# mcdermatt/ICET

Hardware: NVIDIA B200
Metric: registrations/s (64-ch, 75x24 vox, 7 it) (higher is better)
Workload: dtype f32

## Files before the change

### icet_b200/csrc/chunk.cuh

```cuda
#pragma once

thread_local std::string g_err;
int fail(int code, const std::string& msg) {
  g_err = msg;
  return code;
}
#define CK(call)                                                                              \
  do {                                                                                        \
    cudaError_t e_ = (call);                                                                  \
    if (e_ != cudaSuccess)                                                                    \
      return fail(ICET_B200_E_CUDA, std::string(#call) + ": " + cudaGetErrorString(e_));      \
  } while (0)

constexpr int FPB = 21;
constexpr int FP_LIM = (1 << FPB);
constexpr unsigned FULL = 0xffffffffu;
constexpr uint32_t F_STAT1 = 1u;
constexpr uint32_t F_ACTIVE2 = 2u;
constexpr int SORT_SMEM = 4096;
constexpr int NQ = 12;
constexpr int CLUSTER_WARPS = 4;
constexpr int WSORT_MAX = 1024;
constexpr int HUGE_MIN = 32768;
constexpr int HUGE_SLOTS = 64;
constexpr int HUGE_NB = 32768;
constexpr int HUGE_SPLIT = 128;
constexpr uint32_t CLS_CELL = 0x003fffffu;
constexpr uint32_t CLS_IN = 0x00400000u;
constexpr uint32_t CLS_ACTIVE = 0x00800000u;
constexpr uint32_t CLS_NONE = 0x003fffffu;

struct PairDesc {
  const float* s1;
  const float* s2;
  int n1, ld1, n2, ld2;
};

__host__ __device__ __forceinline__ int fp_bits(int n) {
  const unsigned m = (unsigned)(n > 2 ? n : 2) - 1u;
#ifdef __CUDA_ARCH__
  const int lg = 32 - __clz(m);
#else
  const int lg = 32 - __builtin_clz(m);
#endif
  const int b = (62 - lg) / 2;
  return b < 12 ? 12 : (b > 23 ? 23 : b);
}
struct FixPt {
  float fs;
  int fl;
};
// ... 152 lines not shown
  return ok != 0;
}
__device__ __forceinline__ void mbar_wait(unsigned long long* bar, unsigned parity) {
  if (mbar_try_wait(bar, parity)) return;
  unsigned long long t0 = 0;
  for (unsigned spin = 1; !mbar_try_wait(bar, parity); spin++) {
    if ((spin & 1023u) == 0u) {
      unsigned long long t;
      asm volatile("mov.u64 %0, %%globaltimer;" : "=l"(t));
      if (t0 == 0) t0 = t;
      else if (t - t0 > 20000000000ull) __trap();
    }
  }
}

__device__ __forceinline__ uint32_t opaque_u32(uint32_t v) {
  uint32_t r;
  asm volatile("mov.u32 %0, %1;" : "=r"(r) : "r"(v));
  return r;
}
__device__ __forceinline__ float lds_f32(uint32_t a) {
  float v;
  asm volatile("ld.shared.f32 %0, [%1];" : "=f"(v) : "r"(a) : "memory");
  return v;
}
__device__ __forceinline__ uint32_t lds_u32(uint32_t a) {
  uint32_t v;
  asm volatile("ld.shared.u32 %0, [%1];" : "=r"(v) : "r"(a) : "memory");
  return v;
}
__device__ __forceinline__ void sts_u32(uint32_t a, uint32_t v) {
  asm volatile("st.shared.u32 [%0], %1;" ::"r"(a), "r"(v) : "memory");
}
```

### icet_b200/csrc/kernels_pass2.cuh

```cuda
#pragma once

constexpr float INC_MAX_SA = 1.0e-3f;
constexpr float INC_MAX_SB = 0.05f;

struct Pass2Mode {
  bool rebuild;
  int set;
  float fs2;
  int fl2;
  float SA, SB, C;
  const float* trbp;
  unsigned long long* accp;
};

__device__ __forceinline__ float rec2_round_re(float r) {
  return __uint_as_float((__float_as_uint(r * 1.000001f) + 0xffffu) & 0xffff0000u);
}
__device__ __forceinline__ uint2 rec2_pack(float u, float re , uint32_t cls) {
  return make_uint2((__float_as_uint(fmaxf(u, 0.f)) & 0xffffff00u) | (cls & 0xffu), __float_as_uint(re) | (cls >> 8));
}
__device__ __forceinline__ float rec2_u(uint2 v) { return __uint_as_float(v.x & 0xffffff00u); }
__device__ __forceinline__ float rec2_re(uint2 v) { return __uint_as_float(v.y & 0xffff0000u); }
__device__ __forceinline__ uint32_t rec2_cls(uint2 v) { return (v.x & 0xffu) | ((v.y & 0xffffu) << 8); }

// ... 198 lines not shown
  class_move(md.accp, recs, md, old, cls, 0.f, 0.f, 0.f, nz);
  ck.pm[pair].zcls = (int)cls;
}

__device__ __forceinline__ void flush_run2(unsigned long long* accp, int cell, int nb, int nin, int sx, int sy, int sz,
                                           long long pxx, long long pxy, long long pxz, long long pyy, long long pyz,
                                           long long pzz) {
  if (cell < 0) return;
  unsigned long long* q = accp + (size_t)cell * NQ;
  red_add(q, (unsigned long long)nb);
  if (nin == 0) return;
  red_add(q + 1, (unsigned long long)nin);
  red_add(q + 2, (unsigned long long)(long long)sx);
  red_add(q + 3, (unsigned long long)(long long)sy);
  red_add(q + 4, (unsigned long long)(long long)sz);
  red_add(q + 5, (unsigned long long)pxx);
  red_add(q + 6, (unsigned long long)pxy);
  red_add(q + 7, (unsigned long long)pxz);
  red_add(q + 8, (unsigned long long)pyy);
  red_add(q + 9, (unsigned long long)pyz);
  red_add(q + 10, (unsigned long long)pzz);
}

template <int K>
__device__ __forceinline__ void pass2_request_tile(int4* went, const float* src, size_t ld, int cnt, unsigned long long* mbar) {
  float* tx = reinterpret_cast<float*>(went);
  const unsigned bytes = (unsigned)((cnt + 3) & ~3) * 4u;
  mbar_expect_tx(mbar, 3u * bytes);
  bulk_g2s(tx, src, bytes, mbar);
  bulk_g2s(tx + 32 * K, src + ld, bytes, mbar);
  bulk_g2s(tx + 64 * K, src + 2 * ld, bytes, mbar);
}

template <int K, int RD = K, bool ANCH = false>
__device__ __forceinline__ void pass2_warp_tile(const Chunk& ck, int4* went, unsigned long long* mbar, unsigned& mphase,
                                                bool requested, const float* tab, const CellRec* recs, const float* tr,
                                                const Pass2Mode& md, const float* pog, size_t ld, int n, int w0, uint2* mrec,
                                                int* violations, const float4* anch = nullptr) {
  static_assert(K <= 16, "list entries keep the point's index within the tile in 9 bits");
  const int lane = threadIdx.x & 31;
  if (w0 >= n) return;
  const int cnt = min(n - w0, 32 * K);
  const float4* tth = reinterpret_cast<const float4*>(tab);
  const float4* tph = tth + ck.nT + 2;
  const unsigned lt = (1u << lane) - 1u;
  unsigned long long* accp = md.accp;
  const uint32_t sb = opaque_u32(smem_u32(went));
  const uint32_t sbl = sb + 4u * lane;
  constexpr uint32_t PL = 128u * K;
  constexpr uint32_t LO = 3u * PL;
  uint2* rp = mrec + w0;
  if (md.rebuild) {
    if (!requested) {
      __syncwarp();
      if (lane == 0) pass2_request_tile<K>(went, pog + w0, ld, cnt, mbar);
    }
    mbar_wait(mbar, mphase);
    mphase ^= 1u;
    int nact = 0;
#pragma unroll(K % 4 == 0 ? 4 : 2)
    for (int j = 0; j < K; j++) {
      const int li = j * 32 + lane;
      uint32_t cls = 0u;
      if (li < cnt) {
        const float x = lds_f32(sbl + 128u * j), y = lds_f32(sbl + 128u * j + PL), z = lds_f32(sbl + 128u * j + 2u * PL);
        float2 mg;
        point_eval2_fast(ck, tth, tph, recs, tr, 0.f, 0.f, x, y, z, cls, mg);
        if (violations) {
          uint32_t cx;
          float2 mx;
          point_eval2(ck, tth, tph, recs, tr, 0.f, 0.f, x, y, z, cx, mx);
          if (cx != cls) atomicAdd(violations + 1, 1);
        }
        rp[li] = rec2_pack(mg.x, mg.y, cls);
      }
      const bool act = (cls & CLS_ACTIVE) != 0;
      const unsigned am = __ballot_sync(FULL, act);
      if (act) sts_u32(sb + LO + 4u * (nact + __popc(am & lt)), ((uint32_t)li << 23) | (cls & (CLS_CELL | CLS_IN)));
      nact += __popc(am);
    }
    __syncwarp();
    const int q = ((nact + 31) >> 5) | 1;
    const int e0 = lane * q, e1 = min(nact, e0 + q);
    int cur = -1, nb = 0, nin = 0, sx = 0, sy = 0, sz = 0;
    long long pxx = 0, pxy = 0, pxz = 0, pyy = 0, pyz = 0, pzz = 0;
    float ax = 0.f, ay = 0.f, az = 0.f, sc = 0.f;
#pragma unroll 2
    for (int e = e0; e < e1; e++) {
      const unsigned v = lds_u32(sb + LO + 4u * e);
      const int c = (int)(v & CLS_CELL);
      if (c != cur) {
        flush_run2(accp, cur, nb, nin, sx, sy, sz, pxx, pxy, pxz, pyy, pyz, pzz);
        cur = c;
        nb = nin = sx = sy = sz = 0;
        pxx = pxy = pxz = pyy = pyz = pzz = 0;
        if (ANCH) {
          const float4 an = __ldg(anch + cur);
          ax = an.x; ay = an.y; az = an.z; sc = an.w;
        } else {
          vox_anchor2(recs, cur, tr, md.fs2, ax, ay, az, sc);
        }
      }
      nb++;
      if (v & CLS_IN) {
        const uint32_t pa = sb + 4u * (v >> 23);
        int fx, fy, fz;
        fix2(lds_f32(pa), lds_f32(pa + PL), lds_f32(pa + 2u * PL), ax, ay, az, sc, md.fl2, fx, fy, fz);
        nin++;
        sx += fx; sy += fy; sz += fz;
        pxx += (long long)fx * fx; pxy += (long long)fx * fy; pxz += (long long)fx * fz;
        pyy += (long long)fy * fy; pyz += (long long)fy * fz; pzz += (long long)fz * fz;
      }
    }
    flush_run2(accp, cur, nb, nin, sx, sy, sz, pxx, pxy, pxz, pyy, pyz, pzz);
    __syncwarp();
    return;
  }
  int nre = 0;
  constexpr int R = RD;
  static_assert(K % RD == 0, "rows per load group must divide the tile");
#pragma unroll 1
  for (int j0 = 0; j0 < K; j0 += R) {
    uint2 rv[R];
#pragma unroll
    for (int g = 0; g < R; g++) {
      const int li = (j0 + g) * 32 + lane;
      rv[g] = make_uint2(0x7f000000u, 0u);
      if (li < cnt) rv[g] = __ldcg(rp + li);
    }
#pragma unroll
    for (int g = 0; g < R; g++) {
      const int li = (j0 + g) * 32 + lane;
      const bool stable = fmaf(rec2_re(rv[g]), md.SA, md.C) < rec2_u(rv[g]);
      const bool redo = li < cnt && (!stable || violations != nullptr);
      const unsigned rm = __ballot_sync(FULL, redo);
      if (redo) sts_u32(sb + LO + 4u * (nre + __popc(rm & lt)), stable ? ((uint32_t)li | 0x80000000u) : (uint32_t)li);
      nre += __popc(rm);
    }
  }
  if (nre == 0) return;
  const bool staged = nre * 8 > cnt;
  __syncwarp();
  if (staged) {
    if (lane == 0) pass2_request_tile<K>(went, pog + w0, ld, cnt, mbar);
    mbar_wait(mbar, mphase);
    mphase ^= 1u;
  }
  for (int e0 = 0; e0 < nre; e0 += 32) {
    const int e = e0 + lane;
    if (e < nre) {
      const uint32_t le = lds_u32(sb + LO + 4u * e);
      const bool was_stable = (le & 0x80000000u) != 0;
      const int li = (int)(le & 0x7fffffffu);
      float x, y, z;
      if (staged) {
        x = lds_f32(sb + 4u * li); y = lds_f32(sb + 4u * li + PL); z = lds_f32(sb + 4u * li + 2u * PL);
      } else {
        const float* pp = pog + w0 + li;
        x = __ldg(pp); y = __ldg(pp + ld); z = __ldg(pp + 2 * ld);
      }
      const uint32_t old = rec2_cls(__ldcg(rp + li));
      uint32_t cls;
      float2 mg;
      point_eval2_fast(ck, tth, tph, recs, tr, md.SA, md.SB, x, y, z, cls, mg);
      if (violations) {
        uint32_t cx;
        float2 mx;
        point_eval2(ck, tth, tph, recs, tr, md.SA, md.SB, x, y, z, cx, mx);
        if (cx != cls) atomicAdd(violations + 1, 1);
      }
      rp[li] = rec2_pack(mg.x, mg.y, cls);
      if (cls != old) {
        if (was_stable) atomicAdd(violations, 1);
        class_move(accp, recs, md, old, cls, x, y, z, 1);
      }
    }
  }
  __syncwarp();
}

__device__ __forceinline__ void load_pass2_mode(const Chunk& ck, int pair, Pass2Mode& md) {
  const PairMode* pm = ck.pm + pair;
  const int4 h = __ldcg(reinterpret_cast<const int4*>(pm));
  md.rebuild = h.y != 0;
  md.set = h.x;
  const FixPt fp = fix_point(__ldg(&ck.desc[pair].n2));
  md.fs2 = fp.fs;
  md.fl2 = fp.fl;
  md.SA = __int_as_float(h.z);
  md.C = __int_as_float(h.w);
  md.SB = __ldcg(&pm->SB);
  md.trbp = pm->TRb;
  md.accp = ck.acc + ((size_t)h.x * ck.npairs + pair) * ck.ncell * NQ;
}

template <int K = PASS_K, int MINB = PASS_MINB>
__global__ void __launch_bounds__(PASS_THREADS, MINB) k_pass2(const Chunk ck) {
  pdl_prologue();
  extern __shared__ __align__(16) unsigned char smem_raw[];
  __shared__ unsigned long long s_mbar[PASS_WARPS];
  int4* ent = reinterpret_cast<int4*>(smem_raw);
  float* tab = reinterpret_cast<float*>(smem_raw + PASS_WARPS * pass_wslots(K) * 16);
  const int pair = blockIdx.y;
  const int n = ck.n2c[pair];
  const int tile0 = blockIdx.x * pass_tile_points(K);
  if (tile0 >= n && blockIdx.x != 0) return;
  const int warp = threadIdx.x >> 5, lane = threadIdx.x & 31;
  int4* went = ent + warp * pass_wslots(K);
  const int w0 = tile0 + warp * 32 * K;
  const float* pog = ck.pog + (size_t)pair * 3 * ck.n2max;
  Pass2Mode md;
  load_pass2_mode(ck, pair, md);
  if (lane == 0) mbar_init(&s_mbar[warp], 1);
  __syncwarp();
  const bool requested = md.rebuild && w0 < n;
  if (requested && lane == 0) pass2_request_tile<K>(went, pog + w0, (size_t)ck.n2max, min(n - w0, 32 * K), &s_mbar[warp]);
  const float* tabp = ck.binrec;
  if (md.rebuild) {
    const int ntab = pass_tab_floats(ck.nT, ck.nP);
    for (int k = threadIdx.x; k < ntab; k += PASS_THREADS) tab[k] = __ldg(ck.binrec + k);
    tabp = tab;
    __syncthreads();
  }
  float tr[12];
  {
    const float4* tp = reinterpret_cast<const float4*>(ck.TR + (size_t)pair * 12);
    const float4 a = __ldcg(tp), b = __ldcg(tp + 1), c = __ldcg(tp + 2);
    tr[0] = a.x; tr[1] = a.y; tr[2] = a.z; tr[3] = a.w; tr[4] = b.x; tr[5] = b.y; tr[6] = b.z; tr[7] = b.w;
    tr[8] = c.x; tr[9] = c.y; tr[10] = c.z; tr[11] = c.w;
  }
  const CellRec* recs = ck.rec + (size_t)pair * ck.ncell;
  unsigned mphase = 0u;
  pass2_warp_tile<K, K, true>(ck, went, &s_mbar[warp], mphase, requested, tabp, recs, tr, md, pog, (size_t)ck.n2max, n, w0,
                              ck.mrec + (size_t)pair * ck.n2max,
                              (ck.flags & ICET_B200_FLAG_VERIFY_INCREMENTAL) ? &ck.res[pair].reserved[0] : nullptr,
                              ck.anch + (size_t)pair * ck.ncell);
  if (blockIdx.x == 0 && threadIdx.x == 0)
    pass2_dropped_returns(ck, reinterpret_cast<const float4*>(tabp), reinterpret_cast<const float4*>(tabp) + ck.nT + 2, recs,
                          tr, md, pair, ck.nz2[pair]);
}
```

### icet_b200/csrc/kernels_pass.cuh

```cuda
#pragma once
constexpr int PASS_THREADS = 256;
constexpr int PASS_WARPS = PASS_THREADS / 32;
constexpr int PASS_K = 12;
constexpr int PASS_MINB = 4;
constexpr int PASS_K_SMALL = 4;

__host__ __device__ constexpr int pass_wslots(int K) { return 32 * K; }
__host__ __device__ constexpr int pass_tile_points(int K) { return PASS_WARPS * 32 * K; }
__host__ __device__ inline int pass_tab_floats(int nT, int nP) { return 6 * (nT + nP + 4); }
__host__ __device__ inline int pass_smem_bytes(int nT, int nP, int K) {
  return PASS_WARPS * pass_wslots(K) * 16 + pass_tab_floats(nT, nP) * 4;
}

__device__ __forceinline__ int bin_box(float a, const float4* rec, const icet::BinTable& bt, bool& inbox) {
  int k = __float2int_rz(fminf(a, bt.acap) * bt.scale);
  float4 e = rec[k];
  if (a < e.x || a >= e.y) {
    k += (a < e.x) ? -1 : 1;
    e = rec[k];
  }
  inbox = a >= e.z && a <= e.w;
  return k < bt.nb ? k : (k == bt.nb ? 0 : bt.sbin);
}

// ... 70 lines not shown
template <bool SCAN2, int K, int PF = 2, int G = 1>
__device__ __forceinline__ void pass_warp_tile(const Chunk& ck, int4* went ,
                                               const float* tab, const CellRec* recs, const float* tr,
                                               const float* px_, size_t ld, int n, int w0, FixPt fp,
                                               unsigned long long* accp, unsigned long long* dbg_stamp = nullptr,
                                               const int32_t* s1_cell = nullptr, const float* s1_th = nullptr,
                                               const float* s1_ph = nullptr) {
  const int lane = threadIdx.x & 31;
  if (w0 >= n) return;
  const float4* tth = reinterpret_cast<const float4*>(tab);
  const float4* tph = tth + ck.nT + 2;
  const unsigned lt = (1u << lane) - 1u;
  int nin_tile = 0;
  if (!SCAN2) {
    constexpr int R = (K % 4 == 0) ? 4 : ((K % 2 == 0) ? 2 : 1);
#pragma unroll 1
    for (int j0 = 0; j0 < K; j0 += R) {
      int cid[R];
      float rr[R], tt[R], pp[R];
#pragma unroll
      for (int g = 0; g < R; g++) {
        const int i = w0 + (j0 + g) * 32 + lane;
        cid[g] = -1; rr[g] = 0.f; tt[g] = 0.f; pp[g] = 0.f;
        if (i < n) { cid[g] = __ldg(s1_cell + i); rr[g] = __ldg(px_ + i); tt[g] = __ldg(s1_th + i); pp[g] = __ldg(s1_ph + i); }
      }
      float4 ra[R];
#pragma unroll
      for (int g = 0; g < R; g++) {
        ra[g] = make_float4(0.f, 0.f, 0.f, 0.f);
        if (cid[g] >= 0) ra[g] = __ldg(reinterpret_cast<const float4*>(recs + (cid[g] & ~CELL_INBOX)));
      }
#pragma unroll
      for (int g = 0; g < R; g++) {
        const bool in = cid[g] >= 0 && (cid[g] & CELL_INBOX) && (__float_as_uint(ra[g].z) & F_STAT1) && rr[g] >= ra[g].x &&
                        rr[g] <= ra[g].y;
        const unsigned im = __ballot_sync(FULL, in);
        if (in)
          went[nin_tile + __popc(im & lt)] = make_int4(cid[g] & ~CELL_INBOX, __float_as_int(rr[g]), __float_as_int(tt[g]), __float_as_int(pp[g]));
        nin_tile += __popc(im);
      }
    }
  } else if (G > 1) {
    static_assert(G == 1 || K % G == 0, "rows per group must divide the tile");
#pragma unroll 1
    for (int j0 = 0; j0 < K; j0 += G) {
      float gx[G], gy[G], gz[G];
#pragma unroll
      for (int g = 0; g < G; g++) {
        const int i = w0 + (j0 + g) * 32 + lane;
        gx[g] = gy[g] = gz[g] = 0.f;
        if (i < n) { gx[g] = __ldg(px_ + i); gy[g] = __ldg(px_ + ld + i); gz[g] = __ldg(px_ + 2 * ld + i); }
      }
      int gc[G];
      bool gact[G], gin[G];
      float gr[G], gth[G], gph[G];
#pragma unroll
      for (int g = 0; g < G; g++) {
        const int i = w0 + (j0 + g) * 32 + lane;
        gc[g] = -1; gact[g] = false; gin[g] = false; gr[g] = 0.f; gth[g] = 0.f; gph[g] = 0.f;
        if (i < n) point_stage1<SCAN2>(ck, tth, tph, recs, tr, gx[g], gy[g], gz[g], gc[g], gact[g], gin[g], gr[g], gth[g], gph[g]);
      }
#pragma unroll
      for (int g = 0; g < G; g++) {
        const int key = gact[g] ? gc[g] : -1;
        const int prev = __shfl_up_sync(FULL, key, 1);
        const bool head = (lane == 0) || (key != prev);
        const unsigned hm = __ballot_sync(FULL, head);
// ... 301 lines not shown
```

### icet_b200/csrc/kernels_scan1.cuh

```cuda
#pragma once
__device__ __forceinline__ void cell_of(const Chunk& ck, float th, float ph, int& bt, int& bp) {
  bt = icet::bin_lookup(th, ck.bth, 2 * M_PI);
  bp = icet::bin_lookup(ph, ck.bph, M_PI);
}
__device__ __forceinline__ void prep2_compact(const Chunk& ck, int pair, float x, float y, float z, bool keep, bool zero) {
  __shared__ int s_cnt[8], s_zero[8], s_base;
  const int lane = threadIdx.x & 31, warp = threadIdx.x >> 5;
  const unsigned mk = __ballot_sync(FULL, keep), mz = __ballot_sync(FULL, zero);
  if (lane == 0) { s_cnt[warp] = __popc(mk); s_zero[warp] = __popc(mz); }
  __syncthreads();
  if (threadIdx.x == 0) {
    int tot = 0, totz = 0;
    for (int w = 0; w < 8; w++) { const int c = s_cnt[w]; s_cnt[w] = tot; tot += c; totz += s_zero[w]; }
    s_base = tot ? atomicAdd(&ck.n2c[pair], tot) : 0;
    if (totz) atomicAdd(&ck.nz2[pair], totz);
  }
  __syncthreads();
  if (keep) {
    const int o = s_base + s_cnt[warp] + __popc(mk & ((1u << lane) - 1));
    float* pg = ck.pog + (size_t)pair * 3 * ck.n2max;
    pg[o] = x;
    pg[ck.n2max + o] = y;
    pg[2 * (size_t)ck.n2max + o] = z;
  }
// ... 215 lines not shown
  const int lane = threadIdx.x & 31;
  const int total = nz + m;
  auto seq = [&](int i) -> float { return i < nz ? 0.0f : a[i - nz]; };
  int start = 0;
  bool found = false;
  float fi = 0.f, fo = 0.f;
  for (int base = nz; base < total && !found; base += 32) {
    const int i = base + lane;
    bool brk = false;
    if (i < total && i > 0) brk = !(fabsf(seq(i - 1) - seq(i)) <= thresh);
    unsigned mask = __ballot_sync(FULL, brk);
    while (mask && !found) {
      const int pos = base + __ffs(mask) - 1;
      mask &= mask - 1;
      if (pos - start >= n) {
        fi = seq(start) - buff;
        fo = seq(pos - 1) + buff;
        found = true;
      } else {
        start = pos;
      }
    }
  }
  if (!found && total > 0 && total - start >= n) {
    if (seq(start) != 0.0f) {
      fi = seq(start) - buff;
      fo = seq(total - 1) + buff;
    }
  }
  inner = fi;
  outer = fo;
}

__device__ inline void write_cluster_rec(const Chunk& ck, int pair, int cell, int cnt, float inner, float outer) {
  const int bt = cell % ck.nT, bp = cell / ck.nT;
  CellRec rc;
  rc.inner = inner;
  rc.outer = outer;
  rc.cnt1 = cnt;
  rc.flags = ((double)outer > 0.1) ? F_STAT1 : 0u;
  const float azl = ck.azE[bt], azh = ck.azE[bt + 1], ell = ck.elE[bp], elh = ck.elE[bp + 1];
  const float rm = 0.5f * (inner + outer), tm = 0.5f * (azl + azh), pm = 0.5f * (ell + elh);
  icet::s2c(rm, tm, pm, rc.refx, rc.refy, rc.refz);
  float D = (outer - inner) + fabsf(outer) * ((azh - azl) + (elh - ell));
  int e;
  frexpf(fmaxf(D, 1e-20f), &e);
  rc.scale = ldexpf(1.0f, FPB - e - 1);
  ck.rec[(size_t)pair * ck.ncell + cell] = rc;
}

template <int EPL>
__device__ __forceinline__ void warp_sort_regs(float (&v)[EPL]) {
  const int lane = threadIdx.x & 31;
#pragma unroll
  for (int k = 2; k <= 32 * EPL; k <<= 1) {
#pragma unroll
    for (int d = k >> 1; d > 0; d >>= 1) {
      if (d >= EPL) {
        const int ld = d / EPL;
        const bool asc = (k >= 32 * EPL) || ((lane & (k / EPL)) == 0);
        const bool keep_min = (((lane & ld) == 0) == asc);
#pragma unroll
        for (int j = 0; j < EPL; j++) {
          const float o = __shfl_xor_sync(FULL, v[j], ld);
          v[j] = keep_min ? fminf(v[j], o) : fmaxf(v[j], o);
        }
      } else {
#pragma unroll
        for (int j = 0; j < EPL; j++) {
          if ((j & d) == 0) {
            const bool asc = (k >= 32 * EPL) || (k < EPL ? ((j & k) == 0) : ((lane & (k / EPL)) == 0));
            const float lo = fminf(v[j], v[j ^ d]), hi = fmaxf(v[j], v[j ^ d]);
            v[j] = asc ? lo : hi;
            v[j ^ d] = asc ? hi : lo;
          }
        }
      }
    }
  }
}

// ... 169 lines not shown
      if (qm) {
        const int w = __ffs(qm) - 1;
        inner = __shfl_sync(FULL, run_val, w) - buff;
        outer = __shfl_sync(FULL, pmx, w) + buff;
        found = true;
      } else {
        const int nv = min(32, L - e0);
        idx += __shfl_sync(FULL, pc, nv - 1);
        if (bm) {
          const int lb = 31 - __clz(bm);
          start = __shfl_sync(FULL, ie, lb);
          start_val = __shfl_sync(FULL, mn, lb);
        }
        prev_val = __shfl_sync(FULL, mx, nv - 1);
        any_before = true;
      }
    }
    if (!found) {
      seen = idx - nz;
      lo = __float2int_rd(__int_as_float(nxt) * inv_w);
    }
    __syncwarp();
  }
  if (!found && nz + m - start >= n && start_val != 0.0f) {
    inner = start_val - buff;
    outer = prev_val + buff;
  }
  return true;
}

__global__ void __launch_bounds__(CLUSTER_WARPS * 32) k_cluster(const Chunk ck) {
  pdl_prologue();
  const int pair = blockIdx.y;
  constexpr int ROW = WSORT_MAX + WSORT_MAX / 32;
  constexpr int SM_FLOATS = CLUSTER_WARPS * ROW > SORT_SMEM ? CLUSTER_WARPS * ROW : SORT_SMEM;
  constexpr int SM_WORDS = SM_FLOATS > CLUSTER_WARPS * 3 * WB ? SM_FLOATS : CLUSTER_WARPS * 3 * WB;
  __shared__ __align__(16) float s_all[SM_WORDS];
  int* s_bkt = reinterpret_cast<int*>(s_all);
  const int lane = threadIdx.x & 31, warp = threadIdx.x >> 5;
  constexpr int ROW4 = WB_SORT_MAX + WB_SORT_MAX / 32;
  float* srow = s_all + warp * 3 * WB;
  const bool buckets_ok = warp_buckets_ok(ck.thresh);
  const int wmax = warp_cell_max(ck.thresh);
  const int nw = ck.nwork[pair];
  for (int w = blockIdx.x * CLUSTER_WARPS + warp; w < nw; w += gridDim.x * CLUSTER_WARPS) {
    const int cell = ck.work[(size_t)pair * ck.ncell + w];
    const int cnt = ck.cnt1[(size_t)pair * ck.ncell + cell];
    const int nz = ck.cntz[(size_t)pair * ck.ncell + cell];
    const int m = cnt - nz;
    if (m > wmax) continue;
    const float* g = ck.rbuf + (size_t)pair * ck.n1max + ck.off[(size_t)pair * ck.ncell + cell];
    float inner, outer;
    if (m <= WB_SORT_MAX) {
      static_assert(ROW4 <= 3 * WB, "sort row inside the bucket region");
      warp_sort_cell<4>(g, m, srow);
      find_cluster_warp(PaddedRow{srow}, m, nz, ck.n, ck.thresh, ck.buff, inner, outer);
    } else if (!(buckets_ok && find_cluster_buckets_warp(g, m, nz, ck.n, ck.thresh, ck.buff, s_bkt + warp * 3 * WB, inner, outer))) {
      find_cluster_select_warp(g, m, nz, ck.n, ck.thresh, ck.buff, inner, outer);
    }
    if (lane == 0) write_cluster_rec(ck, pair, cell, cnt, inner, outer);
    __syncwarp();
  }
  if (ck.nbig[pair] == 0) return;
  __syncthreads();
  constexpr int NBKT = (SM_FLOATS - 8) / 3;
  int* b_cnt = reinterpret_cast<int*>(s_all);
  int* b_min = b_cnt + NBKT;
  int* b_max = b_min + NBKT;
  int* s_ctl = b_max + NBKT;
  for (int w = blockIdx.x; w < nw; w += gridDim.x) {
    const int cell = ck.work[(size_t)pair * ck.ncell + w];
    const int cnt = ck.cnt1[(size_t)pair * ck.ncell + cell];
    const int nz = ck.cntz[(size_t)pair * ck.ncell + cell];
    const int m = cnt - nz;
    if (m <= wmax) continue;
    if (ck.hbkt) {
      const int hs = ck.hslot[(size_t)pair * ck.ncell + cell];
      if (hs > 0 && ck.hflag[hs - 1] == 0) continue;
    }
    float* g = ck.rbuf + (size_t)pair * ck.n1max + ck.off[(size_t)pair * ck.ncell + cell];
    __syncthreads();
    if (threadIdx.x == 0) s_ctl[0] = 0;
    __syncthreads();
    {
      int mx = 0;
      for (int i0 = threadIdx.x; i0 < m; i0 += 8 * blockDim.x) {
        int v[8];
#pragma unroll
        for (int u = 0; u < 8; u++) {
          const int i = i0 + u * blockDim.x;
          v[u] = i < m ? __float_as_int(g[i]) : 0;
        }
#pragma unroll
        for (int u = 0; u < 8; u++) mx = max(mx, v[u]);
      }
#pragma unroll
      for (int o = 16; o > 0; o >>= 1) mx = max(mx, __shfl_xor_sync(FULL, mx, o));
      if (lane == 0) atomicMax(&s_ctl[0], mx);
    }
    __syncthreads();
    const float rmax = __int_as_float(s_ctl[0]);
    const float wdt = 0.5f * ck.thresh, inv_w = 1.0f / wdt;
    const bool buckets_ok = ck.thresh > 1e-6f && rmax * inv_w < 64.0f * NBKT;
    float inner = 0.f, outer = 0.f;
    if (buckets_ok) {
      int idx = nz, start = 0;
      float start_val = 0.f, prev_val = 0.f;
      bool found = false;
      __syncthreads();
      if (threadIdx.x == 0) { s_ctl[0] = 0; s_ctl[1] = 0; }
      for (int win = 0;; win++) {
        for (int k = threadIdx.x; k < NBKT; k += blockDim.x) { b_cnt[k] = 0; b_min[k] = 0x7f800000; b_max[k] = 0; }
        __syncthreads();
// ... 37 lines not shown
                    found = true;
                    break;
                  }
                  start = idx;
                  start_val = mn;
                }
              } else {
                start_val = mn;
              }
              idx += bc;
              seen += bc;
              prev_val = mxv;
            }
          }
          if (lane == 0) {
            s_ctl[0] += seen;
            if (found || s_ctl[0] >= m) s_ctl[1] = 1;
          }
        }
        __syncthreads();
      }
      if (warp == 0 && !found && nz + m - start >= ck.n && start_val != 0.0f) {
        inner = start_val - ck.buff;
        outer = prev_val + ck.buff;
      }
    } else {
      float* s_r = s_all;
      if (m <= SORT_SMEM) {
        for (int i = threadIdx.x; i < m; i += blockDim.x) s_r[i] = g[i];
        __syncthreads();
        block_sort_asc(s_r, m);
        if (threadIdx.x < 32) find_cluster_warp(s_r, m, nz, ck.n, ck.thresh, ck.buff, inner, outer);
      } else {
        __syncthreads();
        block_sort_asc(g, m);
        if (threadIdx.x < 32) find_cluster_warp(g, m, nz, ck.n, ck.thresh, ck.buff, inner, outer);
      }
    }
    if (threadIdx.x == 0) write_cluster_rec(ck, pair, cell, cnt, inner, outer);
    __syncthreads();
  }
}

__global__ void __launch_bounds__(256) k_huge_init(const Chunk ck) {
  const int slot = blockIdx.y;
  if (slot >= min(*ck.nhuge, HUGE_SLOTS)) return;
  int32_t* t = ck.hbkt + (size_t)slot * 3 * HUGE_NB;
  for (int k = blockIdx.x * blockDim.x + threadIdx.x; k < HUGE_NB; k += gridDim.x * blockDim.x) {
    t[k] = 0;
    t[HUGE_NB + k] = 0x7f800000;
    t[2 * HUGE_NB + k] = 0;
  }
}

__global__ void __launch_bounds__(256) k_huge_hist(const Chunk ck) {
  const int slot = blockIdx.y;
  if (slot >= min(*ck.nhuge, HUGE_SLOTS)) return;
  const int pair = ck.hpair[slot], cell = ck.hcell[slot];
  const size_t ci = (size_t)pair * ck.ncell + cell;
  const int m = ck.cnt1[ci] - ck.cntz[ci];
  const float* g = ck.rbuf + (size_t)pair * ck.n1max + ck.off[ci];
  int32_t* t = ck.hbkt + (size_t)slot * 3 * HUGE_NB;
  const float inv_w = 1.0f / (0.5f * ck.thresh);
  const bool usable = ck.thresh > 1e-6f;
  const int lane = threadIdx.x & 31;
  bool overflow = !usable;
  for (int b0 = (blockIdx.x * blockDim.x + threadIdx.x) & ~31; b0 < m; b0 += gridDim.x * blockDim.x) {
    const int i = b0 + lane;
    int k = -1;
    float r = 0.f;
    if (i < m && usable) {
      r = __ldg(g + i);
// ... 224 lines not shown
```

Before: 91720.

## Add multi-tile ring pass2 kernel with bulk-prefetched match records

Adds k_pass2_ring, where each warp walks several tiles in turn instead of one. In incremental mode it bulk-copies the packed match records into shared memory, and it batches re-evaluation lists across tiles so scattered refreshes are done in full warps. When many points in a tile need re-evaluation it stages their coordinates. The existing pass2 logic is split into reusable helpers, and a vector shared-load helper is added. The aim is to cut launch, per-block setup and global-load latency, at the cost of more shared memory per warp and more serialized work per warp; no host launch change is visible, so whether the new kernel runs is unclear.

```diff
diff --git a/icet_b200/csrc/chunk.cuh b/icet_b200/csrc/chunk.cuh
--- a/icet_b200/csrc/chunk.cuh
+++ b/icet_b200/csrc/chunk.cuh
@@ -235,3 +235,8 @@
 __device__ __forceinline__ void sts_u32(uint32_t a, uint32_t v) {
   asm volatile("st.shared.u32 [%0], %1;" ::"r"(a), "r"(v) : "memory");
 }
+__device__ __forceinline__ uint2 lds_u32x2(uint32_t a) {
+  uint2 v;
+  asm volatile("ld.shared.v2.u32 {%0, %1}, [%2];" : "=r"(v.x), "=r"(v.y) : "r"(a) : "memory");
+  return v;
+}
diff --git a/icet_b200/csrc/kernels_pass2.cuh b/icet_b200/csrc/kernels_pass2.cuh
--- a/icet_b200/csrc/kernels_pass2.cuh
+++ b/icet_b200/csrc/kernels_pass2.cuh
@@ -254,6 +254,122 @@
   bulk_g2s(tx + 64 * K, src + 2 * ld, bytes, mbar);
 }
 
+
+template <int K, bool ANCH>
+__device__ __forceinline__ void pass2_rebuild_staged(const Chunk& ck, uint32_t sb, const float4* tth, const float4* tph,
+                                                     const CellRec* recs, const float* tr, const Pass2Mode& md, uint2* rp,
+                                                     int cnt, int* violations, const float4* anch) {
+  const int lane = threadIdx.x & 31;
+  const unsigned lt = (1u << lane) - 1u;
+  unsigned long long* accp = md.accp;
+  const uint32_t sbl = sb + 4u * lane;
+  constexpr uint32_t PL = 128u * K;
+  constexpr uint32_t LO = 3u * PL;
+  int nact = 0;
+#pragma unroll(K % 4 == 0 ? 4 : 2)
+  for (int j = 0; j < K; j++) {
+    const int li = j * 32 + lane;
+    uint32_t cls = 0u;
+    if (li < cnt) {
+      const float x = lds_f32(sbl + 128u * j), y = lds_f32(sbl + 128u * j + PL), z = lds_f32(sbl + 128u * j + 2u * PL);
+      float2 mg;
+      point_eval2_fast(ck, tth, tph, recs, tr, 0.f, 0.f, x, y, z, cls, mg);
+      if (violations) {
+        uint32_t cx;
+        float2 mx;
+        point_eval2(ck, tth, tph, recs, tr, 0.f, 0.f, x, y, z, cx, mx);
+        if (cx != cls) atomicAdd(violations + 1, 1);
+      }
+      rp[li] = rec2_pack(mg.x, mg.y, cls);
+    }
+    const bool act = (cls & CLS_ACTIVE) != 0;
+    const unsigned am = __ballot_sync(FULL, act);
+    if (act) sts_u32(sb + LO + 4u * (nact + __popc(am & lt)), ((uint32_t)li << 23) | (cls & (CLS_CELL | CLS_IN)));
+    nact += __popc(am);
+  }
+  __syncwarp();
+  const int q = ((nact + 31) >> 5) | 1;
+  const int e0 = lane * q, e1 = min(nact, e0 + q);
+  int cur = -1, nb = 0, nin = 0, sx = 0, sy = 0, sz = 0;
+  long long pxx = 0, pxy = 0, pxz = 0, pyy = 0, pyz = 0, pzz = 0;
+  float ax = 0.f, ay = 0.f, az = 0.f, sc = 0.f;
+#pragma unroll 2
+  for (int e = e0; e < e1; e++) {
+    const unsigned v = lds_u32(sb + LO + 4u * e);
+    const int c = (int)(v & CLS_CELL);
+    if (c != cur) {
+      flush_run2(accp, cur, nb, nin, sx, sy, sz, pxx, pxy, pxz, pyy, pyz, pzz);
+      cur = c;
+      nb = nin = sx = sy = sz = 0;
+      pxx = pxy = pxz = pyy = pyz = pzz = 0;
+      if (ANCH) {
+        const float4 an = __ldg(anch + cur);
+        ax = an.x; ay = an.y; az = an.z; sc = an.w;
+      } else {
+        vox_anchor2(recs, cur, tr, md.fs2, ax, ay, az, sc);
+      }
+    }
+    nb++;
+    if (v & CLS_IN) {
+      const uint32_t pa = sb + 4u * (v >> 23);
+      int fx, fy, fz;
+      fix2(lds_f32(pa), lds_f32(pa + PL), lds_f32(pa + 2u * PL), ax, ay, az, sc, md.fl2, fx, fy, fz);
+      nin++;
+      sx += fx; sy += fy; sz += fz;
+      pxx += (long long)fx * fx; pxy += (long long)fx * fy; pxz += (long long)fx * fz;
+      pyy += (long long)fy * fy; pyz += (long long)fy * fz; pzz += (long long)fz * fz;
+    }
+  }
+  flush_run2(accp, cur, nb, nin, sx, sy, sz, pxx, pxy, pxz, pyy, pyz, pzz);
+  __syncwarp();
+}
+
+__device__ __forceinline__ void pass2_test_row(uint2 rv, int li, int cnt, const Pass2Mode& md, bool verify, uint32_t lst,
+                                               unsigned lt, int& nre, uint32_t base = 0u) {
+  const bool stable = fmaf(rec2_re(rv), md.SA, md.C) < rec2_u(rv);
+  const bool redo = li < cnt && (!stable || verify);
+  const unsigned rm = __ballot_sync(FULL, redo);
+  if (redo) sts_u32(lst + 4u * (nre + __popc(rm & lt)), stable ? ((base + li) | 0x80000000u) : (base + li));
+  nre += __popc(rm);
+}
+
+__device__ __forceinline__ void pass2_eval_listed(const Chunk& ck, const float4* tth, const float4* tph, const CellRec* recs,
+                                                  const float* tr, const Pass2Mode& md, const float* pog, size_t ld, int w0,
+                                                  uint2* rp, uint32_t lst, int nre, bool staged, uint32_t px, uint32_t py,
+                                                  uint32_t pz, int* violations) {
+  const int lane = threadIdx.x & 31;
+  for (int e0 = 0; e0 < nre; e0 += 32) {
+    const int e = e0 + lane;
+    if (e < nre) {
+      const uint32_t le = lds_u32(lst + 4u * e);
+      const bool was_stable = (le & 0x80000000u) != 0;
+      const int li = (int)(le & 0x7fffffffu);
+      float x, y, z;
+      if (staged) {
+        x = lds_f32(px + 4u * li); y = lds_f32(py + 4u * li); z = lds_f32(pz + 4u * li);
+      } else {
+        const float* pp = pog + w0 + li;
+        x = __ldg(pp); y = __ldg(pp + ld); z = __ldg(pp + 2 * ld);
+      }
+      const uint32_t old = rec2_cls(__ldcg(rp + li));
+      uint32_t cls;
+      float2 mg;
+      point_eval2_fast(ck, tth, tph, recs, tr, md.SA, md.SB, x, y, z, cls, mg);
+      if (violations) {
+        uint32_t cx;
+        float2 mx;
+        point_eval2(ck, tth, tph, recs, tr, md.SA, md.SB, x, y, z, cx, mx);
+        if (cx != cls) atomicAdd(violations + 1, 1);
+      }
+      rp[li] = rec2_pack(mg.x, mg.y, cls);
+      if (cls != old) {
+        if (was_stable) atomicAdd(violations, 1);
+        class_move(md.accp, recs, md, old, cls, x, y, z, 1);
+      }
+    }
+  }
+}
+
 template <int K, int RD = K, bool ANCH = false>
 __device__ __forceinline__ void pass2_warp_tile(const Chunk& ck, int4* went, unsigned long long* mbar, unsigned& mphase,
                                                 bool requested, const float* tab, const CellRec* recs, const float* tr,
@@ -266,9 +382,7 @@
   const float4* tth = reinterpret_cast<const float4*>(tab);
   const float4* tph = tth + ck.nT + 2;
   const unsigned lt = (1u << lane) - 1u;
-  unsigned long long* accp = md.accp;
   const uint32_t sb = opaque_u32(smem_u32(went));
-  const uint32_t sbl = sb + 4u * lane;
   constexpr uint32_t PL = 128u * K;
   constexpr uint32_t LO = 3u * PL;
   uint2* rp = mrec + w0;
@@ -279,63 +393,7 @@
     }
     mbar_wait(mbar, mphase);
     mphase ^= 1u;
-    int nact = 0;
-#pragma unroll(K % 4 == 0 ? 4 : 2)
-    for (int j = 0; j < K; j++) {
-      const int li = j * 32 + lane;
-      uint32_t cls = 0u;
-      if (li < cnt) {
-        const float x = lds_f32(sbl + 128u * j), y = lds_f32(sbl + 128u * j + PL), z = lds_f32(sbl + 128u * j + 2u * PL);
-        float2 mg;
-        point_eval2_fast(ck, tth, tph, recs, tr, 0.f, 0.f, x, y, z, cls, mg);
-        if (violations) {
-          uint32_t cx;
-          float2 mx;
-          point_eval2(ck, tth, tph, recs, tr, 0.f, 0.f, x, y, z, cx, mx);
-          if (cx != cls) atomicAdd(violations + 1, 1);
-        }
-        rp[li] = rec2_pack(mg.x, mg.y, cls);
-      }
-      const bool act = (cls & CLS_ACTIVE) != 0;
-      const unsigned am = __ballot_sync(FULL, act);
-      if (act) sts_u32(sb + LO + 4u * (nact + __popc(am & lt)), ((uint32_t)li << 23) | (cls & (CLS_CELL | CLS_IN)));
-      nact += __popc(am);
-    }
-    __syncwarp();
-    const int q = ((nact + 31) >> 5) | 1;
-    const int e0 = lane * q, e1 = min(nact, e0 + q);
-    int cur = -1, nb = 0, nin = 0, sx = 0, sy = 0, sz = 0;
-    long long pxx = 0, pxy = 0, pxz = 0, pyy = 0, pyz = 0, pzz = 0;
-    float ax = 0.f, ay = 0.f, az = 0.f, sc = 0.f;
-#pragma unroll 2
-    for (int e = e0; e < e1; e++) {
-      const unsigned v = lds_u32(sb + LO + 4u * e);
-      const int c = (int)(v & CLS_CELL);
-      if (c != cur) {
-        flush_run2(accp, cur, nb, nin, sx, sy, sz, pxx, pxy, pxz, pyy, pyz, pzz);
-        cur = c;
-        nb = nin = sx = sy = sz = 0;
-        pxx = pxy = pxz = pyy = pyz = pzz = 0;
-        if (ANCH) {
-          const float4 an = __ldg(anch + cur);
-          ax = an.x; ay = an.y; az = an.z; sc = an.w;
-        } else {
-          vox_anchor2(recs, cur, tr, md.fs2, ax, ay, az, sc);
-        }
-      }
-      nb++;
-      if (v & CLS_IN) {
-        const uint32_t pa = sb + 4u * (v >> 23);
-        int fx, fy, fz;
-        fix2(lds_f32(pa), lds_f32(pa + PL), lds_f32(pa + 2u * PL), ax, ay, az, sc, md.fl2, fx, fy, fz);
-        nin++;
-        sx += fx; sy += fy; sz += fz;
-        pxx += (long long)fx * fx; pxy += (long long)fx * fy; pxz += (long long)fx * fz;
-        pyy += (long long)fy * fy; pyz += (long long)fy * fz; pzz += (long long)fz * fz;
-      }
-    }
-    flush_run2(accp, cur, nb, nin, sx, sy, sz, pxx, pxy, pxz, pyy, pyz, pzz);
-    __syncwarp();
+    pass2_rebuild_staged<K, ANCH>(ck, sb, tth, tph, recs, tr, md, rp, cnt, violations, anch);
     return;
   }
   int nre = 0;
@@ -351,14 +409,7 @@
       if (li < cnt) rv[g] = __ldcg(rp + li);
     }
 #pragma unroll
-    for (int g = 0; g < R; g++) {
-      const int li = (j0 + g) * 32 + lane;
-      const bool stable = fmaf(rec2_re(rv[g]), md.SA, md.C) < rec2_u(rv[g]);
-      const bool redo = li < cnt && (!stable || violations != nullptr);
-      const unsigned rm = __ballot_sync(FULL, redo);
-      if (redo) sts_u32(sb + LO + 4u * (nre + __popc(rm & lt)), stable ? ((uint32_t)li | 0x80000000u) : (uint32_t)li);
-      nre += __popc(rm);
-    }
+    for (int g = 0; g < R; g++) pass2_test_row(rv[g], (j0 + g) * 32 + lane, cnt, md, violations != nullptr, sb + LO, lt, nre);
   }
   if (nre == 0) return;
   const bool staged = nre * 8 > cnt;
@@ -368,36 +419,7 @@
     mbar_wait(mbar, mphase);
     mphase ^= 1u;
   }
-  for (int e0 = 0; e0 < nre; e0 += 32) {
-    const int e = e0 + lane;
-    if (e < nre) {
-      const uint32_t le = lds_u32(sb + LO + 4u * e);
-      const bool was_stable = (le & 0x80000000u) != 0;
-      const int li = (int)(le & 0x7fffffffu);
-      float x, y, z;
-      if (staged) {
-        x = lds_f32(sb + 4u * li); y = lds_f32(sb + 4u * li + PL); z = lds_f32(sb + 4u * li + 2u * PL);
-      } else {
-        const float* pp = pog + w0 + li;
-        x = __ldg(pp); y = __ldg(pp + ld); z = __ldg(pp + 2 * ld);
-      }
-      const uint32_t old = rec2_cls(__ldcg(rp + li));
-      uint32_t cls;
-      float2 mg;
-      point_eval2_fast(ck, tth, tph, recs, tr, md.SA, md.SB, x, y, z, cls, mg);
-      if (violations) {
-        uint32_t cx;
-        float2 mx;
-        point_eval2(ck, tth, tph, recs, tr, md.SA, md.SB, x, y, z, cx, mx);
-        if (cx != cls) atomicAdd(violations + 1, 1);
-      }
-      rp[li] = rec2_pack(mg.x, mg.y, cls);
-      if (cls != old) {
-        if (was_stable) atomicAdd(violations, 1);
-        class_move(accp, recs, md, old, cls, x, y, z, 1);
-      }
-    }
-  }
+  pass2_eval_listed(ck, tth, tph, recs, tr, md, pog, ld, w0, rp, sb + LO, nre, staged, sb, sb + PL, sb + 2u * PL, violations);
   __syncwarp();
 }
 
@@ -416,7 +438,21 @@
   md.accp = ck.acc + ((size_t)h.x * ck.npairs + pair) * ck.ncell * NQ;
 }
 
-template <int K = PASS_K, int MINB = PASS_MINB>
+__device__ __forceinline__ const float* pass2_tables(const Chunk& ck, const Pass2Mode& md, float* tab) {
+  if (!md.rebuild) return ck.binrec;
+  const int ntab = pass_tab_floats(ck.nT, ck.nP);
+  for (int k = threadIdx.x; k < ntab; k += PASS_THREADS) tab[k] = __ldg(ck.binrec + k);
+  __syncthreads();
+  return tab;
+}
+__device__ __forceinline__ void load_tr(const Chunk& ck, int pair, float* tr) {
+  const float4* tp = reinterpret_cast<const float4*>(ck.TR + (size_t)pair * 12);
+  const float4 a = __ldcg(tp), b = __ldcg(tp + 1), c = __ldcg(tp + 2);
+  tr[0] = a.x; tr[1] = a.y; tr[2] = a.z; tr[3] = a.w; tr[4] = b.x; tr[5] = b.y; tr[6] = b.z; tr[7] = b.w;
+  tr[8] = c.x; tr[9] = c.y; tr[10] = c.z; tr[11] = c.w;
+}
+
+template <int K, int MINB>
 __global__ void __launch_bounds__(PASS_THREADS, MINB) k_pass2(const Chunk ck) {
   pdl_prologue();
   extern __shared__ __align__(16) unsigned char smem_raw[];
@@ -437,20 +473,9 @@
   __syncwarp();
   const bool requested = md.rebuild && w0 < n;
   if (requested && lane == 0) pass2_request_tile<K>(went, pog + w0, (size_t)ck.n2max, min(n - w0, 32 * K), &s_mbar[warp]);
-  const float* tabp = ck.binrec;
-  if (md.rebuild) {
-    const int ntab = pass_tab_floats(ck.nT, ck.nP);
-    for (int k = threadIdx.x; k < ntab; k += PASS_THREADS) tab[k] = __ldg(ck.binrec + k);
-    tabp = tab;
-    __syncthreads();
-  }
+  const float* tabp = pass2_tables(ck, md, tab);
   float tr[12];
-  {
-    const float4* tp = reinterpret_cast<const float4*>(ck.TR + (size_t)pair * 12);
-    const float4 a = __ldcg(tp), b = __ldcg(tp + 1), c = __ldcg(tp + 2);
-    tr[0] = a.x; tr[1] = a.y; tr[2] = a.z; tr[3] = a.w; tr[4] = b.x; tr[5] = b.y; tr[6] = b.z; tr[7] = b.w;
-    tr[8] = c.x; tr[9] = c.y; tr[10] = c.z; tr[11] = c.w;
-  }
+  load_tr(ck, pair, tr);
   const CellRec* recs = ck.rec + (size_t)pair * ck.ncell;
   unsigned mphase = 0u;
   pass2_warp_tile<K, K, true>(ck, went, &s_mbar[warp], mphase, requested, tabp, recs, tr, md, pog, (size_t)ck.n2max, n, w0,
@@ -461,3 +486,120 @@
     pass2_dropped_returns(ck, reinterpret_cast<const float4*>(tabp), reinterpret_cast<const float4*>(tabp) + ck.nT + 2, recs,
                           tr, md, pair, ck.nz2[pair]);
 }
+
+#ifndef PASS2_TV
+#define PASS2_TV 4
+#endif
+#ifndef PASS2_STAGE_HEAVY
+#define PASS2_STAGE_HEAVY 1
+#endif
+constexpr int PASS2_T = PASS2_TV;
+constexpr int PASS2_WBYTES = pass_wslots(PASS_K) * 16 + 128;
+__host__ __device__ constexpr int pass2_span_points() { return PASS2_T * pass_tile_points(PASS_K); }
+__host__ __device__ inline int pass2_smem_bytes(int nT, int nP) { return PASS_WARPS * PASS2_WBYTES + pass_tab_floats(nT, nP) * 4; }
+
+__device__ __forceinline__ void pass2_request_recs(void* dst, const uint2* src, int cnt, unsigned long long* mbar) {
+  const unsigned bytes = (unsigned)((cnt + 1) & ~1) * 8u;
+  mbar_expect_tx(mbar, bytes);
+  bulk_g2s(dst, src, bytes, mbar);
+}
+
+__global__ void __launch_bounds__(PASS_THREADS, PASS_MINB) k_pass2_ring(const Chunk ck) {
+  constexpr int K = PASS_K, T = PASS2_T;
+  constexpr uint32_t LO = 3u * 128u * K;
+  constexpr int WSTEP = PASS_WARPS * 32 * K;
+  static_assert(LO + 4u * (32 * K + 32) <= (uint32_t)PASS2_WBYTES, "warp scratch too small for the carried-over list");
+  static_assert(T * WSTEP < (1 << 30), "list entries keep the point's offset from the warp's first tile in 30 bits");
+  extern __shared__ __align__(16) unsigned char smem_raw[];
+  __shared__ unsigned long long s_mbar[PASS_WARPS];
+  float* tab = reinterpret_cast<float*>(smem_raw + PASS_WARPS * PASS2_WBYTES);
+  const int pair = blockIdx.y;
+  const int n = ck.n2c[pair];
+  if (blockIdx.x * pass2_span_points() >= n && blockIdx.x != 0) return;
+  const int warp = threadIdx.x >> 5, lane = threadIdx.x & 31;
+  int4* went = reinterpret_cast<int4*>(smem_raw + warp * PASS2_WBYTES);
+  unsigned long long* mbar = &s_mbar[warp];
+  const size_t ld = (size_t)ck.n2max;
+  const float* pog = ck.pog + (size_t)pair * 3 * ld;
+  uint2* mrec = ck.mrec + (size_t)pair * ld;
+  const int wb = blockIdx.x * pass2_span_points() + warp * 32 * K;
+  Pass2Mode md;
+  load_pass2_mode(ck, pair, md);
+  if (lane == 0) mbar_init(mbar, 1);
+  __syncwarp();
+  if (lane == 0 && wb < n) {
+    if (md.rebuild) pass2_request_tile<K>(went, pog + wb, ld, min(n - wb, 32 * K), mbar);
+    else pass2_request_recs(went, mrec + wb, min(n - wb, 32 * K), mbar);
+  }
+  const float* tabp = pass2_tables(ck, md, tab);
+  const float4* tth = reinterpret_cast<const float4*>(tabp);
+  const float4* tph = tth + ck.nT + 2;
+  __shared__ float s_tr[12];
+  if (threadIdx.x < 12) s_tr[threadIdx.x] = __ldcg(ck.TR + (size_t)pair * 12 + threadIdx.x);
+  __syncthreads();
+  const CellRec* recs = ck.rec + (size_t)pair * ck.ncell;
+  int* violations = (ck.flags & ICET_B200_FLAG_VERIFY_INCREMENTAL) ? &ck.res[pair].reserved[0] : nullptr;
+  const uint32_t sb = opaque_u32(smem_u32(went));
+  const unsigned lt = (1u << lane) - 1u;
+  unsigned mphase = 0u;
+  if (md.rebuild) {
+    float tr[12];
+    load_tr(ck, pair, tr);
+#pragma unroll 1
+    for (int t = 0, w0 = wb; t < T && w0 < n; t++, w0 += WSTEP) {
+      const int cnt = min(n - w0, 32 * K);
+      if (t > 0 && lane == 0) pass2_request_tile<K>(went, pog + w0, ld, cnt, mbar);
+      mbar_wait(mbar, mphase);
+      mphase ^= 1u;
+      pass2_rebuild_staged<K, true>(ck, sb, tth, tph, recs, tr, md, mrec + w0, cnt, violations,
+                                    ck.anch + (size_t)pair * ck.ncell);
+    }
+  } else {
+    int nre = 0;
+#pragma unroll 1
+    for (int t = 0, w0 = wb; t < T && w0 < n; t++, w0 += WSTEP) {
+      const int cnt = min(n - w0, 32 * K);
+      mbar_wait(mbar, mphase);
+      mphase ^= 1u;
+      uint2 rv[K];
+#pragma unroll
+      for (int g = 0; g < K; g++) {
+        const int li = g * 32 + lane;
+        rv[g] = li < cnt ? lds_u32x2(sb + 8u * li) : make_uint2(0x7f000000u, 0u);
+      }
+      __syncwarp();
+      const int w1 = w0 + WSTEP;
+      const bool more = t + 1 < T && w1 < n;
+#if !PASS2_STAGE_HEAVY
+      if (lane == 0 && more) pass2_request_recs(went, mrec + w1, min(n - w1, 32 * K), mbar);
+#endif
+      const int nre0 = nre;
+#pragma unroll
+      for (int g = 0; g < K; g++)
+        pass2_test_row(rv[g], g * 32 + lane, cnt, md, violations != nullptr, sb + LO, lt, nre, (uint32_t)(w0 - wb));
+#if PASS2_STAGE_HEAVY
+      if ((nre - nre0) * 8 > cnt) {
+        __syncwarp();
+        if (lane == 0) pass2_request_tile<K>(went, pog + w0, ld, cnt, mbar);
+        if (nre0 > 0)
+          pass2_eval_listed(ck, tth, tph, recs, s_tr, md, pog, ld, wb, mrec + wb, sb + LO, nre0, false, 0u, 0u, 0u, violations);
+        mbar_wait(mbar, mphase);
+        mphase ^= 1u;
+        const uint32_t sx = sb - 4u * (uint32_t)(w0 - wb);
+        pass2_eval_listed(ck, tth, tph, recs, s_tr, md, pog, ld, wb, mrec + wb, sb + LO + 4u * nre0, nre - nre0, true, sx,
+                          sx + 128u * K, sx + 256u * K, violations);
+        nre = 0;
+        __syncwarp();
+      }
+      if (lane == 0 && more) pass2_request_recs(went, mrec + w1, min(n - w1, 32 * K), mbar);
+#endif
+      if (nre >= 32 || (!more && nre > 0)) {
+        __syncwarp();
+        pass2_eval_listed(ck, tth, tph, recs, s_tr, md, pog, ld, wb, mrec + wb, sb + LO, nre, false, 0u, 0u, 0u, violations);
+        nre = 0;
+        __syncwarp();
+      }
+    }
+  }
+  if (blockIdx.x == 0 && threadIdx.x == 0) pass2_dropped_returns(ck, tth, tph, recs, s_tr, md, pair, ck.nz2[pair]);
+}
```

After: 90780 (median of 6 runs). 0.99x the previous value.

## Fuse per-cell first-scan statistics accumulation into the cluster kernel

Applied to the files above, without the earlier changes.

After computing a cell's cluster bounds, the cluster kernel now immediately accumulates that cell's fixed-point moment sums (count, first and second moments) from the gathered per-cell points, and marks the record with a new done flag. The later pass kernel then skips those points, which avoids a second scattered read of them. It also prefetches the cell's gathered arrays into L2 while sorting, and sorts large cells in a scratch copy so the gathered radii stay intact for the stats. The cost is extra work and shared-memory staging inside the cluster kernel, and a risk of imbalance for cells with many points.

```diff
diff --git a/icet_b200/csrc/chunk.cuh b/icet_b200/csrc/chunk.cuh
--- a/icet_b200/csrc/chunk.cuh
+++ b/icet_b200/csrc/chunk.cuh
@@ -17,6 +17,7 @@
 constexpr unsigned FULL = 0xffffffffu;
 constexpr uint32_t F_STAT1 = 1u;
 constexpr uint32_t F_ACTIVE2 = 2u;
+constexpr uint32_t F_STAT1_DONE = 4u;
 constexpr int SORT_SMEM = 4096;
 constexpr int NQ = 12;
 constexpr int CLUSTER_WARPS = 4;
diff --git a/icet_b200/csrc/kernels_pass.cuh b/icet_b200/csrc/kernels_pass.cuh
--- a/icet_b200/csrc/kernels_pass.cuh
+++ b/icet_b200/csrc/kernels_pass.cuh
@@ -126,7 +126,8 @@
       }
 #pragma unroll
       for (int g = 0; g < R; g++) {
-        const bool in = cid[g] >= 0 && (cid[g] & CELL_INBOX) && (__float_as_uint(ra[g].z) & F_STAT1) && rr[g] >= ra[g].x &&
+        const bool in = cid[g] >= 0 && (cid[g] & CELL_INBOX) &&
+                        (__float_as_uint(ra[g].z) & (F_STAT1 | F_STAT1_DONE)) == F_STAT1 && rr[g] >= ra[g].x &&
                         rr[g] <= ra[g].y;
         const unsigned im = __ballot_sync(FULL, in);
         if (in)
diff --git a/icet_b200/csrc/kernels_scan1.cuh b/icet_b200/csrc/kernels_scan1.cuh
--- a/icet_b200/csrc/kernels_scan1.cuh
+++ b/icet_b200/csrc/kernels_scan1.cuh
@@ -271,7 +271,7 @@
   outer = fo;
 }
 
-__device__ inline void write_cluster_rec(const Chunk& ck, int pair, int cell, int cnt, float inner, float outer) {
+__device__ inline CellRec cluster_rec(const Chunk& ck, int cell, int cnt, float inner, float outer) {
   const int bt = cell % ck.nT, bp = cell / ck.nT;
   CellRec rc;
   rc.inner = inner;
@@ -285,7 +285,81 @@
   int e;
   frexpf(fmaxf(D, 1e-20f), &e);
   rc.scale = ldexpf(1.0f, FPB - e - 1);
-  ck.rec[(size_t)pair * ck.ncell + cell] = rc;
+  return rc;
+}
+
+__device__ inline void write_cluster_rec(const Chunk& ck, int pair, int cell, int cnt, float inner, float outer) {
+  ck.rec[(size_t)pair * ck.ncell + cell] = cluster_rec(ck, cell, cnt, inner, outer);
+}
+
+constexpr int STAT1_BATCH = 512;
+__device__ __forceinline__ void point_stage2(float r, float th, float ph, float refx, float refy, float refz, float sc,
+                                             int lim, int& fx, int& fy, int& fz);
+
+__device__ __forceinline__ void prefetch_l2_words(const void* p, int m) {
+  const int lane = threadIdx.x & 31;
+  const uintptr_t a1 = (uintptr_t)p + 4 * (size_t)m;
+  for (uintptr_t a = ((uintptr_t)p & ~(uintptr_t)127) + 128 * lane; a < a1; a += 32 * 128)
+    asm volatile("prefetch.global.L2 [%0];" ::"l"(a));
+}
+
+__device__ inline void cell_stat1_warp(const float* __restrict__ r, const int32_t* __restrict__ cid, const float* __restrict__ th,
+                                       const float* __restrict__ ph, int m, int first, int step, const CellRec& rc,
+                                       FixPt fp, float* stage, unsigned long long* accp) {
+  const int lane = threadIdx.x & 31;
+  const unsigned lt = (1u << lane) - 1u;
+  const float sc = rc.scale * fp.fs;
+  int nin = 0;
+  long long v[9] = {0, 0, 0, 0, 0, 0, 0, 0, 0};
+  for (int b0 = first * STAT1_BATCH; b0 < m; b0 += step * STAT1_BATCH) {
+    int ns = 0;
+    constexpr int R = 4;
+#pragma unroll 1
+    for (int j0 = 0; j0 < STAT1_BATCH && b0 + j0 < m; j0 += 32 * R) {
+      int c[R];
+      float rr[R], tt[R], pp[R];
+#pragma unroll
+      for (int g = 0; g < R; g++) {
+        const int i = b0 + j0 + 32 * g + lane;
+        c[g] = 0; rr[g] = 0.f; tt[g] = 0.f; pp[g] = 0.f;
+        if (i < m) { c[g] = __ldg(cid + i); rr[g] = __ldg(r + i); tt[g] = __ldg(th + i); pp[g] = __ldg(ph + i); }
+      }
+#pragma unroll
+      for (int g = 0; g < R; g++) {
+        const bool in = (c[g] & CELL_INBOX) && rr[g] >= rc.inner && rr[g] <= rc.outer;
+        const unsigned im = __ballot_sync(FULL, in);
+        if (in) {
+          const int e = ns + __popc(im & lt);
+          stage[e] = rr[g];
+          stage[STAT1_BATCH + e] = tt[g];
+          stage[2 * STAT1_BATCH + e] = pp[g];
+        }
+        ns += __popc(im);
+      }
+    }
+    __syncwarp();
+    for (int e = lane; e < ns; e += 32) {
+      int fx, fy, fz;
+      point_stage2(stage[e], stage[STAT1_BATCH + e], stage[2 * STAT1_BATCH + e], rc.refx, rc.refy, rc.refz, sc, fp.fl, fx,
+                   fy, fz);
+      nin++;
+      v[0] += fx; v[1] += fy; v[2] += fz;
+      v[3] += (long long)fx * fx; v[4] += (long long)fx * fy; v[5] += (long long)fx * fz;
+      v[6] += (long long)fy * fy; v[7] += (long long)fy * fz; v[8] += (long long)fz * fz;
+    }
+    __syncwarp();
+  }
+  nin = __reduce_add_sync(FULL, nin);
+  if (nin == 0) return;
+#pragma unroll
+  for (int o = 16; o > 0; o >>= 1)
+#pragma unroll
+    for (int k = 0; k < 9; k++) v[k] += __shfl_xor_sync(FULL, v[k], o);
+  if (lane == 0) {
+    red_add(accp + 1, (unsigned long long)nin);
+#pragma unroll
+    for (int k = 0; k < 9; k++) red_add(accp + 2 + k, (unsigned long long)v[k]);
+  }
 }
 
 template <int EPL>
@@ -521,6 +595,9 @@
 __global__ void __launch_bounds__(CLUSTER_WARPS * 32) k_cluster(const Chunk ck) {
   pdl_prologue();
   const int pair = blockIdx.y;
+  const size_t o1 = (size_t)pair * ck.n1max;
+  const FixPt fp = fix_point(ck.desc[pair].n1);
+  unsigned long long* accp = ck.acc + (size_t)pair * ck.ncell * NQ;
   constexpr int ROW = WSORT_MAX + WSORT_MAX / 32;
   constexpr int SM_FLOATS = CLUSTER_WARPS * ROW > SORT_SMEM ? CLUSTER_WARPS * ROW : SORT_SMEM;
   constexpr int SM_WORDS = SM_FLOATS > CLUSTER_WARPS * 3 * WB ? SM_FLOATS : CLUSTER_WARPS * 3 * WB;
@@ -538,7 +615,9 @@
     const int nz = ck.cntz[(size_t)pair * ck.ncell + cell];
     const int m = cnt - nz;
     if (m > wmax) continue;
-    const float* g = ck.rbuf + (size_t)pair * ck.n1max + ck.off[(size_t)pair * ck.ncell + cell];
+    const size_t og = o1 + ck.off[(size_t)pair * ck.ncell + cell];
+    const float* g = ck.rbuf + og;
+    prefetch_l2_words(ck.cellg + og, m); prefetch_l2_words(ck.thg + og, m); prefetch_l2_words(ck.phg + og, m);
     float inner, outer;
     if (m <= WB_SORT_MAX) {
       static_assert(ROW4 <= 3 * WB, "sort row inside the bucket region");
@@ -547,8 +626,13 @@
     } else if (!(buckets_ok && find_cluster_buckets_warp(g, m, nz, ck.n, ck.thresh, ck.buff, s_bkt + warp * 3 * WB, inner, outer))) {
       find_cluster_select_warp(g, m, nz, ck.n, ck.thresh, ck.buff, inner, outer);
     }
-    if (lane == 0) write_cluster_rec(ck, pair, cell, cnt, inner, outer);
+    CellRec rc = cluster_rec(ck, cell, cnt, inner, outer);
+    if (rc.flags & F_STAT1) rc.flags |= F_STAT1_DONE;
+    if (lane == 0) ck.rec[(size_t)pair * ck.ncell + cell] = rc;
     __syncwarp();
+    static_assert(3 * STAT1_BATCH <= 3 * WB, "stage inside the warp's bucket region");
+    if (rc.flags & F_STAT1)
+      cell_stat1_warp(g, ck.cellg + og, ck.thg + og, ck.phg + og, m, 0, 1, rc, fp, srow, accp + (size_t)cell * NQ);
   }
   if (ck.nbig[pair] == 0) return;
   __syncthreads();
@@ -567,7 +651,8 @@
       const int hs = ck.hslot[(size_t)pair * ck.ncell + cell];
       if (hs > 0 && ck.hflag[hs - 1] == 0) continue;
     }
-    float* g = ck.rbuf + (size_t)pair * ck.n1max + ck.off[(size_t)pair * ck.ncell + cell];
+    const size_t og = o1 + ck.off[(size_t)pair * ck.ncell + cell];
+    const float* g = ck.rbuf + og;
     __syncthreads();
     if (threadIdx.x == 0) s_ctl[0] = 0;
     __syncthreads();
@@ -671,12 +756,24 @@
         block_sort_asc(s_r, m);
         if (threadIdx.x < 32) find_cluster_warp(s_r, m, nz, ck.n, ck.thresh, ck.buff, inner, outer);
       } else {
+        float* s_g = ck.r1 + og;
+        for (int i = threadIdx.x; i < m; i += blockDim.x) s_g[i] = g[i];
         __syncthreads();
-        block_sort_asc(g, m);
-        if (threadIdx.x < 32) find_cluster_warp(g, m, nz, ck.n, ck.thresh, ck.buff, inner, outer);
-      }
-    }
-    if (threadIdx.x == 0) write_cluster_rec(ck, pair, cell, cnt, inner, outer);
+        block_sort_asc(s_g, m);
+        if (threadIdx.x < 32) find_cluster_warp(s_g, m, nz, ck.n, ck.thresh, ck.buff, inner, outer);
+      }
+    }
+    if (threadIdx.x == 0) { s_ctl[2] = __float_as_int(inner); s_ctl[3] = __float_as_int(outer); }
+    __syncthreads();
+    CellRec rc = cluster_rec(ck, cell, cnt, __int_as_float(s_ctl[2]), __int_as_float(s_ctl[3]));
+    __syncthreads();
+    const bool stat1 = (rc.flags & F_STAT1) && !ck.hbkt;
+    if (stat1) rc.flags |= F_STAT1_DONE;
+    if (threadIdx.x == 0) ck.rec[(size_t)pair * ck.ncell + cell] = rc;
+    static_assert(CLUSTER_WARPS * 3 * WB <= SM_WORDS, "stages inside the block's shared memory");
+    if (stat1)
+      cell_stat1_warp(g, ck.cellg + og, ck.thg + og, ck.phg + og, m, warp, CLUSTER_WARPS, rc, fp, s_all + warp * 3 * WB,
+                      accp + (size_t)cell * NQ);
     __syncthreads();
   }
 }
```

Measured after the change: 91680 before, 95100 after, median of 6. 1.04x the previous value.
